# BauerLab/VARSCOT

Hardware: AMD Instinct MI355X
Metric: guides/sec (candidate sites/sec alongside) at <=8 mismatches on a 3.0 Gbp reference (higher is better)
Workload: dtype u32

## Files before the change

varscot_amd/csrc/vsc_api.cpp:

```cpp
#include <algorithm>
#include <atomic>
#include <chrono>
#include <cstdlib>
#include <cmath>
#include <cstdio>
#include <cstring>
#include <memory>
#include <new>
#include <string>
#include <vector>

#include "vsc_bulge.h"
#include "vsc_efficiency.h"
#include "vsc_pattern.h"
#include "vsc_pattern_enum.h"
#include "vsc_pattern_bulge.h"
#include "vsc_enum.h"
#include "vsc_internal.h"
#include "vsc_objects.h"
#include "vsc_pairs.h"
#include "vsc_pick_device.h"
#include "vsc_sites.h"
#include "vsc_bulge_table.h"
#include "vsc_table.h"
// ... 1275 lines not shown
                double e2 = 0;
                for (int left = 0; left <= (int)m; ++left) e2 += (double)left_reads[c][left] * neighbours(left - k0 - k1 - 2);
                const double per_list = e2 / kBucketsPerSeg;
                bytes += (1.0 - std::exp(-per_list)) * (double)genome->ix_class_sites[c] * block_bytes;
                visits += per_list * (double)genome->ix_class_chunks[c] / kSegments;
            }
            for (int k : {k0, k1}) {
                const double per_list = (double)reads_any * neighbours(k) / kBucketsPerSeg;
                bytes += (1.0 - std::exp(-per_list)) * sites_all * block_bytes;
                visits += per_list * chunks_all;
            }
            cost[cut] = std::max(bytes / 4.2e12, visits * 215.0 / ((double)n_cus * 4 * 2.0e9));
        }
        int best = -1;
        for (int cut = 0; cut < 9; ++cut)
            if (cost[cut] >= 0 && (best < 0 || cost[cut] < cost[best])) best = cut;
        const int forced = dbg.seed_tight >= 1 ? dbg.seed_tight - 1 : -1;
        if (forced >= 0 && forced < 9 && cost[forced] >= 0) best = forced;
        if (best < 0) best = 4 * (int)(m ? (m - 1) / kSegments : 0u);
        plan.k0 = (uint32_t)(best % 3);
        plan.k1 = (uint32_t)(best / 3);
        *k2_max = std::min<int>(2, (int)m - (int)plan.k0 - (int)plan.k1 - 2);
    }
    plan.n_nbr = neighbours(std::max<int>(std::max<int>((int)plan.k0, (int)plan.k1), *k2_max));
    return plan;
}

hipError_t seed_plan(vsc_ctx *ctx, const vsc_genome *genome, const uint32_t *gp, uint32_t n_guides, const PassFound &f, SeedArgs &sa,
                     int *n_groups, bool *shared)
{
    int k2_max = 0;
    const SeedPlan plan = seed_cut(genome, gp, n_guides, f.max_mm, ctx->n_cus, ctx->dbg, &k2_max);
    const uint64_t n_pairs = (uint64_t)n_guides * (neighbours((int)plan.k0) + neighbours((int)plan.k1) + plan.n_pam * neighbours(k2_max));
    const uint64_t list_cap = n_pairs + (uint64_t)kLists * (kGuideUnroll - 1) + 2 * kGuideUnroll;
    VSC_TRY(ctx->seed_off.ensure((kLists + 1) * sizeof(uint32_t)));
    VSC_TRY(ctx->seed_poff.ensure((kLists + 1) * sizeof(uint32_t)));
    VSC_TRY(ctx->seed_lrest.ensure(list_cap * sizeof(uint2)));
    VSC_TRY(hipMemsetAsync(ctx->seed_lrest.p, 0xFF, list_cap * sizeof(uint2), ctx->stream));
    VSC_TRY(launch_seed_lists((const uint2 *)ctx->guides.p, n_guides, plan, (uint32_t *)ctx->seed_off.p, (uint32_t *)ctx->seed_poff.p,
                              (uint2 *)ctx->seed_lrest.p, ctx->stream));
    VSC_TRY(hipEventRecord(ctx->ev[kEvPrepEnd], ctx->stream));
    sa.chunk_tab = genome->d_ix_chunk_tab;
    sa.n_chunks = genome->ix_chunks;
    sa.vert = genome->d_ix_vert;
    sa.list_rest = (const uint2 *)ctx->seed_lrest.p;
    sa.sites = genome->d_ix_sites;
    sa.edge_bits = genome->d_ix_edge;
    sa.guides = (const uint2 *)ctx->guides.p;
    sa.poff = (const uint32_t *)ctx->seed_poff.p;
    sa.max_mm = f.max_mm;
    sa.k_half = f.max_mm / 2;
    sa.k_seg0 = plan.k0;
    sa.k_seg1 = plan.k1;
    sa.contig_end = genome->d_contig_end;
    sa.n_contigs = genome->n_contigs;
    sa.counters = (unsigned long long *)ctx->counters.p;
    sa.n_parts = (uint32_t)f.n_parts;
    uint32_t groups_per_cu = kSlicedWavesPerSimd;
    if (ctx->dbg.seed_groups_per_cu) groups_per_cu = ctx->dbg.seed_groups_per_cu;
    *shared = (uint64_t)n_guides * neighbours((int)std::max(plan.k0, plan.k1)) / kBucketsPerSeg >= 72;
    if (ctx->dbg.seed_shared >= 0) *shared = ctx->dbg.seed_shared == 1;
    const uint32_t n_grabs = (sa.n_chunks + kSlicedGrab - 1) / kSlicedGrab;
    const uint32_t n_waves_max = (uint32_t)ctx->n_cus * groups_per_cu * kWavesPerGroup;
    const uint32_t n_waves = std::max<uint32_t>(1, std::min<uint32_t>(n_waves_max, *shared ? n_grabs * kWavesPerGroup : n_grabs));
    *n_groups = (int)((n_waves + kWavesPerGroup - 1) / kWavesPerGroup);
    sa.group_out = *shared && ctx->dbg.seed_group_out != 0 ? 1u : 0u;
    const uint32_t owners = sa.group_out ? (uint32_t)*n_groups : (uint32_t)*n_groups * kWavesPerGroup;
    const uint64_t per_wave = f.cap / ((uint64_t)owners * 8 * f.n_parts);
    uint32_t want_reserve = (uint32_t)std::min<uint64_t>(f.n_parts > 8 ? (sa.group_out ? 1024 : 128) : 1024, std::max<uint64_t>(kWave, per_wave));
    if (ctx->dbg.seed_reserve) want_reserve = std::min<uint32_t>(1024, std::max<uint32_t>(kWave, ctx->dbg.seed_reserve));
    sa.reserve_log2 = 6;
    while ((2u << sa.reserve_log2) <= want_reserve) ++sa.reserve_log2;
    sa.reserve = 1u << sa.reserve_log2;
    sa.pos_pad = f.pos_pad;
    sa.pos_base = f.pos_base;
    uint64_t part_cap = f.cap / f.n_parts + f.cap / f.n_parts / 7 + 4096;
    part_cap = std::max<uint64_t>(part_cap, (uint64_t)(1.2 * genome->seen_rate[f.max_mm] * std::min<uint32_t>(n_guides, kRegionReads)) + 4096);
    sa.part_cap = part_cap + (uint64_t)owners * sa.reserve;
    return hipSuccess;
}

constexpr uint32_t kSeedPartsDefault = 1;
constexpr uint32_t kSeedPartsMax = 64;
constexpr uint32_t kSeedPartGroupsPerCu = 3;
constexpr uint64_t kSeedPartMinRecords = 1ull << 27;

uint32_t plan_parts(vsc_ctx *ctx, const vsc_genome *genome, const PassFound &f, const SeedArgs &sa, uint32_t n_guides, bool shared, SortLevel1 &l1)
{
    const vsc_debug_params &dbg = ctx->dbg;
    uint32_t want = dbg.seed_parts ? dbg.seed_parts : kSeedPartsDefault;
    if (want <= 1 || !shared || ctx->cu_masked || dbg.sort_optimistic == 0 || !genome->sort_slots_ok[f.max_mm]) return 1;
    const double rate = genome->seen_rate[f.max_mm];
    const uint64_t n_max = (uint64_t)(rate * std::min<uint32_t>(n_guides, kRegionReads)), n_all = (uint64_t)(rate * n_guides);
    want = std::min<uint32_t>({want, std::max<uint32_t>(1, sa.n_chunks), kSeedPartsMax});
    if (!dbg.seed_parts && n_all < (uint64_t)want * kSeedPartMinRecords) return 1;
    uint64_t sort_cap, slot_cap;
    unsigned max_bits;
    sort_limits(dbg, &sort_cap, &max_bits, &slot_cap);
    unsigned bits = level_bits(n_max, sort_cap, max_bits, f.key_bits, (size_t)f.n_parts);
    if (bits == 0) {
        if (!dbg.seed_parts) return 1;
        bits = 1;
    }
    if (dbg.sort_optimistic != 1 && !slots_fit((uint64_t)f.n_parts << bits, slot_cap, std::max<uint64_t>(n_all, 1), ctx->keys_b.cap, 0, false)) return 1;
    l1.bits = bits;
    l1.slot_cap = slot_cap;
    return want;
}

size_t round256(size_t n) { return (n + 255) / 256 * 256; }

hipError_t search_in_parts(vsc_ctx *ctx, PassFound &f, const SeedArgs &all, uint32_t K, bool shared, unsigned long long *cnt, size_t cnt_bytes,
                           uint32_t *list_total, float *scan_ms)
{
    const hipStream_t A = ctx->stream;
    SeedArgs sa = all;
    const uint32_t R = (uint32_t)f.n_parts;
    const size_t cnt_at = 0, segs_at = round256(cnt_bytes), tile_at = segs_at + round256(R * sizeof(SortSeg));
    const size_t stride = tile_at + round256((R + 1) * sizeof(uint32_t)), dev_stride = stride - segs_at;
    if (!ctx->stream_b) VSC_TRY(hipStreamCreateWithFlags(&ctx->stream_b, hipStreamNonBlocking));
    const hipStream_t B = ctx->stream_b;
    while (ctx->part_ev.size() < 3 * (size_t)K + 1) {
        hipEvent_t e = nullptr;
        VSC_TRY(hipEventCreate(&e));
        ctx->part_ev.push_back(e);
    }
    if (ctx->pinned_cap < K * stride + 256) {
        if (ctx->pinned) (void)hipHostFree(ctx->pinned);
        ctx->pinned = nullptr;
        ctx->pinned_cap = 0;
        VSC_TRY(hipHostMalloc(&ctx->pinned, K * stride + 256, hipHostMallocDefault));
        ctx->pinned_cap = K * stride + 256;
    }
    char *const pin = (char *)ctx->pinned;
    uint32_t *const pin_total = (uint32_t *)(pin + K * stride);
    SortLevel1 &l1 = f.l1;
    const size_t n_bins = (size_t)R << l1.bits;
    VSC_TRY(ctx->keys_b.ensure(std::max<uint64_t>((uint64_t)n_bins * l1.slot_cap, f.cap) * sizeof(uint64_t)));
    VSC_TRY(ctx->sort_tabs.ensure(3 * n_bins * sizeof(uint32_t)));
    VSC_TRY(ctx->sort_over.ensure(256 + n_bins * sizeof(SortSeg)));
    VSC_TRY(ctx->sort_segs.ensure(std::max<size_t>(K * dev_stride, round256(R * sizeof(SortSeg)) + (R + 1) * sizeof(uint32_t))));
    SortArgs pa{};
    pa.n_segs = R;
    pa.in = (const uint64_t *)ctx->keys_a.p;
    pa.out = (uint64_t *)ctx->keys_b.p;
    pa.cursor = (uint32_t *)ctx->sort_tabs.p + n_bins;
    pa.hist = pa.cursor;
    pa.bin_start = pa.cursor + n_bins;
    pa.bin_bits = l1.bits;
    pa.bin_shift = kRecPosShift + f.pos_pad + f.key_bits - l1.bits;
    pa.fill = l1.fill;
    pa.fill_shift = l1.fill_shift;
    pa.slot_cap = (uint32_t)l1.slot_cap;
    pa.overflow = (uint32_t *)ctx->sort_over.p + 2;
    VSC_TRY(hipMemsetAsync(pa.cursor, 0, n_bins * sizeof(uint32_t), A));
    VSC_TRY(hipMemsetAsync(ctx->sort_over.p, 0, 3 * sizeof(uint32_t), A));
    VSC_TRY(hipMemcpyAsync(pin_total, (const uint32_t *)ctx->seed_poff.p + kLists, sizeof(uint32_t), hipMemcpyDeviceToHost, A));
    VSC_TRY(hipEventRecord(ctx->ev[kEvSearchStart], A));
    for (uint32_t i = 0; i < K; ++i) {
        const uint32_t chunk_first = (uint32_t)((uint64_t)all.n_chunks * i / K);
        sa.chunk_tab = all.chunk_tab + chunk_first;
        sa.n_chunks = (uint32_t)((uint64_t)all.n_chunks * (i + 1) / K) - chunk_first;
        const uint32_t per_cu = ctx->dbg.seed_groups_per_cu ? ctx->dbg.seed_groups_per_cu : (i ? kSeedPartGroupsPerCu : (uint32_t)kSlicedWavesPerSimd);
        const uint32_t n_grabs = (sa.n_chunks + kSlicedGrab - 1) / kSlicedGrab;
        const uint32_t n_waves = std::max<uint32_t>(1, std::min<uint32_t>((uint32_t)ctx->n_cus * per_cu * kWavesPerGroup, shared ? n_grabs * kWavesPerGroup : n_grabs));
        if (i) VSC_TRY(hipMemsetAsync(sa.counters + kCursorBase, 0, (size_t)kCursors * kCursorStride * sizeof(unsigned long long), A));
        VSC_TRY(hipEventRecord(ctx->part_ev[3 * i], A));
        VSC_TRY(launch_seed_sliced(sa, (int)((n_waves + kWavesPerGroup - 1) / kWavesPerGroup), shared, A));
        VSC_TRY(hipEventRecord(ctx->part_ev[3 * i + 1], A));
        VSC_TRY(hipMemcpyAsync(pin + i * stride + cnt_at, sa.counters, cnt_bytes, hipMemcpyDeviceToHost, A));
        VSC_TRY(hipEventRecord(ctx->part_ev[3 * i + 2], A));
    }
    VSC_TRY(hipEventRecord(ctx->ev[kEvSearchEnd], A));
    bool lost = false;
    for (uint32_t i = 0; i < K; ++i) {
        VSC_TRY(hipEventSynchronize(ctx->part_ev[3 * i + 2]));
        const unsigned long long *const now = (const unsigned long long *)(pin + i * stride + cnt_at);
        const unsigned long long *const before = i ? (const unsigned long long *)(pin + (i - 1) * stride + cnt_at) : nullptr;
        if (now[kCntOverflow]) lost = true;
        if (lost) continue;
        SortSeg *const segs = (SortSeg *)(pin + i * stride + segs_at);
        uint32_t *const tile0 = (uint32_t *)(pin + i * stride + tile_at);
        uint64_t tiles = 0;
        for (uint32_t q = 0; q < R; ++q) {
            const uint64_t b = before ? before[kCntPart + 4 * q] : 0, e = now[kCntPart + 4 * q];
            const uint64_t at = (uint64_t)q * sa.part_cap + b;
            segs[q] = SortSeg{at, at, 0, (uint32_t)(e - b), 0, q, 0};
            tile0[q] = (uint32_t)tiles;
            tiles += (e - b + kSortTile - 1) / kSortTile;
        }
        tile0[R] = (uint32_t)tiles;
        if (tiles == 0) continue;
        if (tiles >= (1ull << 31)) return hipErrorInvalidValue;
        char *const dev = (char *)ctx->sort_segs.p + i * dev_stride;
        VSC_TRY(hipStreamWaitEvent(B, ctx->part_ev[3 * i + 2], 0));
        VSC_TRY(hipMemcpyAsync(dev, segs, dev_stride, hipMemcpyHostToDevice, B));
        pa.segs = (const SortSeg *)dev;
        pa.seg_tile0 = (const uint32_t *)(dev + (tile_at - segs_at));
        pa.n_tiles = (uint32_t)tiles;
        pa.xcd_tiles = 0;
        pa.xcd_by_region = 0;
        if (ctx->dbg.sort_xcd != 0 && tiles >= 64) {
            pa.xcd_by_region = 1;
            for (uint32_t x = 0; x <= 8; ++x) pa.xcd_first[x] = tile0[(uint64_t)R * x / 8];
            for (uint32_t x = 0; x < 8; ++x) pa.xcd_tiles = std::max(pa.xcd_tiles, pa.xcd_first[x + 1] - pa.xcd_first[x]);
        }
        VSC_TRY(launch_bin_partition(pa, B));
    }
    VSC_TRY(hipEventRecord(ctx->part_ev[3 * K], B));
    VSC_TRY(hipStreamWaitEvent(A, ctx->part_ev[3 * K], 0));
    std::memcpy(cnt, pin + (K - 1) * stride + cnt_at, cnt_bytes);
    *list_total = *pin_total;
    *scan_ms = 0;
    for (uint32_t i = 0; i < K; ++i) {
        float ms = 0;
        VSC_TRY(hipEventElapsedTime(&ms, ctx->part_ev[3 * i], ctx->part_ev[3 * i + 1]));
        *scan_ms += ms;
    }
    l1.done = !lost;
    if (lost) VSC_TRY(hipStreamSynchronize(A));
    return hipSuccess;
}

int find_pass(vsc_ctx *ctx, const vsc_genome *genome, const uint64_t *guides, uint32_t n_guides, uint32_t guide_base,
              const vsc_search_params *params, bool keep_bases, bool sort_only, vsc_timing &t, PassFound &f)
{
    const int algo = (int)t.algorithm;
    const uint32_t m = params->max_mismatches;
    f.algo = algo;
    f.max_mm = m;
    f.guide_base = guide_base;
    f.bases = keep_bases;
    const uint32_t n_pad = (n_guides + kGuideUnroll - 1) / kGuideUnroll * kGuideUnroll;
    std::vector<uint32_t> gp((size_t)(n_pad + kGuideUnroll) * 2, 0xFFFFFFFFu);
    for (uint32_t i = 0; i < n_guides; ++i) guide_planes(guides[i], &gp[2 * (size_t)i], &gp[2 * (size_t)i + 1]);
    VSC_HIP(ctx, ctx->guides.ensure(gp.size() * sizeof(uint32_t)));
    VSC_HIP(ctx, ctx->counters.ensure(kCounterWords * sizeof(unsigned long long)));
    VSC_HIP(ctx, hipEventRecord(ctx->ev[kEvPassStart], ctx->stream));
    VSC_HIP(ctx, hipMemcpyAsync(ctx->guides.p, gp.data(), gp.size() * sizeof(uint32_t), hipMemcpyHostToDevice, ctx->stream));

    const double own_bases = (double)genome->n_tiles * kTileBases;
    const double sites_est = genome->sites ? (double)genome->sites : own_bases / 4;
    f.cap = (uint64_t)(1.5 * sites_est * n_guides * hit_probability(m)) + (1u << 20);
    const double seen_rate = genome->seen_rate[m];
    if (algo == VSC_ALGO_SCAN) f.cap = std::max<uint64_t>(f.cap, (uint64_t)(1.2 * seen_rate * n_guides) + 4096);
    unsigned long long cnt[kCntPart + 4 * kParts] = {};
    f.n_parts = (int)((n_guides + kRegionReads - 1) / kRegionReads);
    f.pos_base = (uint32_t)(genome->first_word * 32);
    const unsigned pos_bits = std::max(1u, ceil_log2((uint64_t)genome->dev_words * 32));
    f.pos_pad = pos_bits < 32 ? 32 - pos_bits : 0;
    f.key_bits = pos_bits + 1 + ceil_log2(std::min<uint32_t>(n_guides, kRegionReads));

    ScanArgs a{};
    SeedArgs sa{};
    int n_groups = 1;
    bool seed_shared = false;
    const bool use_fill = algo == VSC_ALGO_SEED && sort_only && !keep_bases;
    uint32_t n_parts_k = 1;
    auto owners_of = [](const SeedArgs &s, int groups) { return (uint64_t)(s.group_out ? groups : groups * kWavesPerGroup); };
    if (algo == VSC_ALGO_SCAN) {
        fill_pam(a, params);
        fill_genome(a, ctx, genome);
        a.guides = (const uint4 *)ctx->guides.p;
        a.n_guides_padded = n_pad;
        a.max_mm = m;
        a.k_half = m / 2;
        n_groups = scan_groups(ctx, a.n_tiles);
        t.genome_bytes += (uint64_t)genome->n_tiles * kTileWords * 3 * sizeof(uint32_t);
        VSC_HIP(ctx, hipEventRecord(ctx->ev[kEvPrepEnd], ctx->stream));
    } else {
        VSC_HIP(ctx, seed_plan(ctx, genome, gp.data(), n_guides, f, sa, &n_groups, &seed_shared));
        if (use_fill) {
// ... 7073 lines not shown
```

varscot_amd/csrc/vsc_internal.h:

```cpp
#pragma once

#include <hip/hip_runtime.h>
#include <stdint.h>

#include "varscot_hip.h"
#include "vsc_efficiency.h"
#include "vsc_eff_trees.h"
#include "vsc_mh.h"
#include "vsc_fold.h"
#include "vsc_edit.h"
#include "vsc_variation.h"
#include "vsc_prime.h"
#include "vsc_hdr.h"
#include "vsc_effects.h"

namespace vsc {

constexpr int kWave = 64;
constexpr int kWavesPerGroup = 4;
constexpr int kSitesPerLane = 8;
constexpr int kBatch = kWave * kSitesPerLane;
constexpr int kQueueCap = kBatch + kWave;
constexpr int kHitCap = 128;
constexpr int kTileWords = kWave;
constexpr int kTileBases = kTileWords * 32;
constexpr int kChunkTiles = 8;
constexpr int kGuideUnroll = 4;
constexpr uint32_t kMask23 = 0x7FFFFFu;
constexpr int kSiteStrandBit = 23;
constexpr int kSiteEdgeBit = 24;
constexpr uint32_t kPadWords = 4;

constexpr int kSegments = 3;
constexpr int kSegBases = 7;
constexpr int kBucketsPerSeg = 1 << (2 * kSegBases);
constexpr int kBuckets = kSegments * kBucketsPerSeg;
constexpr int kSeedHitCap = 256;
constexpr int kSlicedSites = 32;
constexpr int kSlicedChunk = kWave * kSlicedSites;
constexpr int kRestBases = VSC_READ_LEN - kSegBases;
constexpr int kCmpBases = 2 * kSegBases;
constexpr int kVertWords = 2 * kCmpBases;
constexpr int kSeedClasses = 3;
constexpr int kLists = (kSegments - 1 + kSeedClasses) * kBucketsPerSeg;
constexpr int kListBudgetShift = 16;
constexpr uint32_t kListNoBudget = 15;
constexpr int kTokLaneShift = 26;
constexpr int kTokSlotShift = 14;
constexpr uint32_t kTokReadMask = (1u << kTokSlotShift) - 1u;
constexpr int kSlicedResolve = 3;
constexpr int kSlicedTokCap = 512;
constexpr uint32_t kChunkBucketMask = 0xFFFFu;
constexpr int kChunkMinusShift = 16;
constexpr int kChunkEdgeBit = 28;
constexpr int kChunkClassShift = 29;
constexpr uint32_t kIndexLayout = 2;
constexpr int kSlicedWavesPerSimd = 6;
constexpr int kSlicedGrab = 8;

enum { kCntHits = 0, kCntChunk = 1, kCntSites = 2, kCntOverflow = 3, kCntVisited = 4, kCntPad = 5, kCntLost = 6, kCntGroups = 7, kCntSlots = 8 };
constexpr int kRegionBits = 6;
constexpr int kRegionReads = 1 << kRegionBits;
constexpr int kParts = 256;
constexpr int kMaxPassReads = kParts * kRegionReads;
constexpr int kCntPart = 8;
constexpr int kCursors = 32;
constexpr int kCursorStride = 16;
constexpr int kCursorBase = kCntPart + 4 * kParts + 8;
constexpr int kCounterWords = kCursorBase + kCursors * kCursorStride;

constexpr int kRecPosShift = 23;
constexpr int kRecStrandShift = 55;
constexpr int kRecReadShift = 56;
constexpr int kRecKeyBits = 33 + kRegionBits;
constexpr uint64_t kRecSentinel = ~0ull;

constexpr int kSortThreads = 512;
constexpr int kSortItems = 16;
constexpr int kSortTile = kSortThreads * kSortItems;
constexpr int kFinThreads = 512;
constexpr int kFinItems = 16;
constexpr int kSortCap = kFinThreads * kFinItems - 128;
constexpr int kSortMaxBinBits = 11;
constexpr int kSortSubBits = 13;
constexpr int kSortSubBitsRows = 12;
constexpr int kHistTiles = 8;

struct PamMasks {
    uint32_t ah, al;
    uint32_t bh, bl;
};

struct ScanArgs {
    const uint32_t *hi, *lo, *nm;
    uint32_t first_pos;
    uint32_t n_tiles;
    const uint4 *guides;
    uint32_t n_guides_padded;
    uint32_t max_mm;
    uint32_t k_half;
    uint32_t n_pam;
    PamMasks pam[3];
    const uint32_t *contig_end;
    uint32_t n_contigs;
    uint64_t *hit_keys;
    uint32_t *hit_vals;
    unsigned long long hit_cap;
    unsigned long long *counters;
    uint32_t *site_x, *site_l, *site_pos;
};

struct SortSeg {
    uint64_t in_off;
    uint64_t out_off;
    uint64_t final_off;
    uint32_t n_in;
    uint32_t guide_base;
    uint32_t region = 0;
    uint32_t pad = 0;
};

struct SortArgs {
    const SortSeg *segs;
    const uint32_t *seg_tile0;
    uint32_t n_segs, n_tiles;
    const uint64_t *in;
    const uint64_t *pair_keys;
    const uint32_t *pair_vals;
    uint64_t *out;
    const uint32_t *side_in;
    uint32_t *side_out;
    uint32_t *hist;
    uint32_t *cursor;
    uint32_t *bin_start;
    uint32_t bin_bits, bin_shift;
    uint32_t pos_pad;
    uint32_t pos_base;
    uint32_t xcd_tiles;
    uint32_t xcd_by_region;
    uint32_t xcd_first[9];
    const uint32_t *fill;
    uint32_t fill_shift;
    uint32_t slot_cap;
    uint32_t *overflow;
};

struct FinArgs {
    const SortSeg *segs;
    uint32_t n_segs;
    const uint64_t *src;
    const uint32_t *hist;
    const uint32_t *bin_start;
    uint32_t bin_bits;
    uint32_t sub_shift, sub_bits;
    uint32_t low_bits;
    uint32_t pos_pad;
    uint32_t pos_base;
    SortSeg *over;
    uint32_t over_cap;
    uint32_t cap;
    uint32_t *n_over;
    uint32_t *cursor;
    const uint32_t *contig_off;
    uint32_t n_contigs;
    vsc_hit *out;
    uint32_t slot_cap;
    const uint32_t *overflow;
    const uint32_t *side_src;
    const uint2 *guides;
    uint32_t guide_first;
    uint4 *rows;
    uint64_t rows_first;
};

struct ScoreArgs {
    const vsc_hit *hits;
    uint64_t n;
    const uint2 *hl;
    uint32_t first_pos;
    uint64_t n_plane_words;
    const uint32_t *contig_off;
    const uint2 *guides;
    double *mit;
    uint8_t *mit_flags;
    uint8_t *features;
    const uint64_t *seg_prefix;
    const uint64_t *seg_start;
    uint32_t n_segs;
};

struct SeedPlan {
    uint32_t max_mm, k0, k1, tight;
    uint32_t n_nbr;
    uint32_t n_pam;
    uint32_t pam_codes;
};

struct SeedArgs {
    const uint4 *chunk_tab;
    const uint32_t *vert;
    const uint2 *list_rest;
    const uint2 *sites;
    const uint32_t *edge_bits;
    const uint2 *guides;
    uint32_t n_chunks;
    const uint32_t *poff;
    uint32_t max_mm, k_half;
    uint32_t k_seg0, k_seg1;
    const uint32_t *contig_end;
    uint32_t n_contigs;
    uint64_t *hit_recs;
    uint32_t *hit_side;
    uint32_t group_out;
    uint32_t reserve;
    uint32_t reserve_log2;
    uint32_t pos_pad;
    uint32_t pos_base;
    uint32_t n_parts;
    unsigned long long part_cap;
    unsigned long long *counters;
    uint32_t *fill;
};

constexpr int kSumThreads = 256;
constexpr int kSumItems = 8;
constexpr int kSumTile = kSumThreads * kSumItems;
constexpr int kSumTilesPerBlock = 8;
// ... 569 lines not shown
```

varscot_amd/csrc/vsc_sort.hip:

```cpp
#include "vsc_internal.h"
#include "vsc_device.h"

namespace vsc {

namespace {

constexpr int kLaneRun = 2;
__device__ __forceinline__ uint32_t tile_record(int k, uint32_t t)
{
    return (uint32_t)(k / kLaneRun) * (uint32_t)(kLaneRun * kSortThreads) + t * (uint32_t)kLaneRun + (uint32_t)(k % kLaneRun);
}

template <int kThreads>
__device__ __forceinline__ uint32_t block_exclusive_scan(uint32_t *s, uint32_t n, uint32_t *s_wave)
{
    const uint32_t t = threadIdx.x, lane = t % kWave, wave = t / kWave;
    const uint32_t per = n > (uint32_t)kThreads ? n / kThreads : 1u;
    const bool mine = t * per < n;
    uint32_t v[4] = {0u, 0u, 0u, 0u};
    uint32_t sum = 0;
    if (mine)
        for (uint32_t i = 0; i < per; ++i) {
            v[i] = s[t * per + i];
            sum += v[i];
        }
    uint32_t inc = sum;
#pragma unroll
    for (int d = 1; d < kWave; d <<= 1) {
        const uint32_t o = __shfl_up(inc, d, kWave);
        if (lane >= (uint32_t)d) inc += o;
    }
    if (lane == kWave - 1) s_wave[wave] = inc;
    block_sync();
    uint32_t before = 0, total = 0;
#pragma unroll
    for (int w = 0; w < kThreads / kWave; ++w) {
        const uint32_t x = s_wave[w];
        before += (uint32_t)w < wave ? x : 0u;
        total += x;
    }
    uint32_t run = before + inc - sum;
    if (mine)
        for (uint32_t i = 0; i < per; ++i) {
            s[t * per + i] = run;
            run += v[i];
        }
    block_sync();
    return total;
}

__device__ __forceinline__ bool slot_filled(const SortArgs &a, uint64_t at, uint32_t held)
{
    return ((uint32_t)at & ((1u << a.fill_shift) - 1u)) < held;
}

__device__ __forceinline__ uint64_t pack_pair(uint64_t key, uint32_t val, uint32_t pos_pad, uint32_t pos_base)
{
    const uint64_t high = (key >> 32) & ((1ull << (kRecKeyBits - 32)) - 1ull);
    return (((high << 32) | (uint32_t)(((uint32_t)key - pos_base) << pos_pad)) << kRecPosShift) | (val & kMask23);
}

}

template <bool kPairs, bool kFill = false>
__global__ __launch_bounds__(kSortThreads) void bin_hist_kernel(const SortArgs a)
{
    __shared__ uint32_t s_hist[1 << kSortMaxBinBits];
    const uint32_t t = threadIdx.x;
    const uint32_t nbins = 1u << a.bin_bits;
    for (uint32_t b = t; b < nbins; b += kSortThreads) s_hist[b] = 0;
    block_sync();
    const uint32_t tile_begin = blockIdx.x * kHistTiles, tile_end = min(tile_begin + (uint32_t)kHistTiles, a.n_tiles);
    uint32_t seg = segment_of_tile(a.seg_tile0, a.n_segs, tile_begin);
    for (uint32_t tile = tile_begin; tile < tile_end; ++tile) {
        if (tile >= a.seg_tile0[seg + 1]) {
            block_sync();
            for (uint32_t b = t; b < nbins; b += kSortThreads) {
                const uint32_t c = s_hist[b];
                if (c) atomicAdd(&a.hist[((size_t)a.segs[seg].region << a.bin_bits) + b], c);
                s_hist[b] = 0;
            }
            block_sync();
            seg = segment_of_tile(a.seg_tile0, a.n_segs, tile);
        }
        const SortSeg sg = a.segs[seg];
        const uint32_t first = (tile - a.seg_tile0[seg]) * (uint32_t)kSortTile;
        const uint32_t n = min(sg.n_in - first, (uint32_t)kSortTile);
        uint64_t r[kSortItems];
        uint32_t held[kFill ? kSortItems / kLaneRun : 1];
        if (kFill) {
#pragma unroll
            for (int j = 0; j < kSortItems / kLaneRun; ++j) {
                const uint32_t i = tile_record(j * kLaneRun, t);
                held[j] = a.fill[(sg.in_off + first + (i < n ? i : 0u)) >> a.fill_shift];
            }
        }
#pragma unroll
        for (int k = 0; k < kSortItems; ++k) {
            const uint32_t i = tile_record(k, t);
            const bool valid = i < n && (!kFill || slot_filled(a, sg.in_off + first + i, held[kFill ? k / kLaneRun : 0]));
            const uint64_t at = sg.in_off + first + (valid ? i : 0u);
            const uint64_t v = kPairs ? a.pair_keys[at] : a.in[at];
            r[k] = valid ? v : kRecSentinel;
        }
#pragma unroll
        for (int k = 0; k < kSortItems; ++k) {
            if (kPairs) {
                if (tile_record(k, t) < n) atomicAdd(&s_hist[(uint32_t)(r[k] >> a.bin_shift)], 1u);
            } else {
                if (!(r[k] >> 63)) atomicAdd(&s_hist[(uint32_t)(r[k] >> a.bin_shift) & (nbins - 1u)], 1u);
            }
        }
    }
    block_sync();
    for (uint32_t b = t; b < nbins; b += kSortThreads) {
        const uint32_t c = s_hist[b];
        if (c) atomicAdd(&a.hist[((size_t)a.segs[seg].region << a.bin_bits) + b], c);
    }
}

hipError_t launch_bin_hist(const SortArgs &args, hipStream_t stream)
{
    if (args.n_tiles == 0) return hipSuccess;
    const unsigned blocks = (args.n_tiles + kHistTiles - 1) / kHistTiles;
    if (args.pair_keys)
        hipLaunchKernelGGL(bin_hist_kernel<true>, dim3(blocks), dim3(kSortThreads), 0, stream, args);
    else if (args.fill)
        hipLaunchKernelGGL((bin_hist_kernel<false, true>), dim3(blocks), dim3(kSortThreads), 0, stream, args);
    else
        hipLaunchKernelGGL(bin_hist_kernel<false>, dim3(blocks), dim3(kSortThreads), 0, stream, args);
    return hipGetLastError();
}

__global__ __launch_bounds__(512) void bin_scan_kernel(const SortArgs a)
{
    __shared__ uint32_t s_cnt[1 << kSortMaxBinBits];
    __shared__ uint32_t s_wave[512 / kWave];
    const uint32_t nbins = 1u << a.bin_bits;
    const size_t base = (size_t)blockIdx.x << a.bin_bits;
    for (uint32_t b = threadIdx.x; b < nbins; b += 512) s_cnt[b] = a.hist[base + b];
    block_sync();
    block_exclusive_scan<512>(s_cnt, nbins, s_wave);
    for (uint32_t b = threadIdx.x; b < nbins; b += 512) {
        a.bin_start[base + b] = s_cnt[b];
        if (!a.slot_cap) a.cursor[base + b] = s_cnt[b];
    }
}

hipError_t launch_bin_scan(const SortArgs &args, hipStream_t stream)
{
    if (args.n_segs == 0) return hipSuccess;
    hipLaunchKernelGGL(bin_scan_kernel, dim3(args.n_segs), dim3(512), 0, stream, args);
    return hipGetLastError();
}

template <bool kPairs, bool kSide = false, bool kFill = false>
__global__ __launch_bounds__(kSortThreads) void bin_partition_kernel(const SortArgs a)
{
    __shared__ uint64_t s_rec[kSortTile];
    __shared__ uint32_t s_cnt[(1 << kSortMaxBinBits) + kWave];
    __shared__ uint32_t s_gbase[kPairs ? (1 << kSortMaxBinBits) : 1];
    __shared__ uint32_t s_over[(1 << kSortMaxBinBits) / 32 + 1];
    __shared__ uint32_t s_wave[kSortThreads / kWave];
    const uint32_t t = threadIdx.x;
    const uint32_t nbins = 1u << a.bin_bits;
    uint32_t tile = blockIdx.x;
    if (a.xcd_by_region) {
        tile = a.xcd_first[blockIdx.x & 7u] + (blockIdx.x >> 3);
        if (tile >= a.xcd_first[(blockIdx.x & 7u) + 1u]) return;
    } else if (a.xcd_tiles) {
        tile = (blockIdx.x & 7u) * a.xcd_tiles + (blockIdx.x >> 3);
        if ((blockIdx.x >> 3) >= a.xcd_tiles || tile >= a.n_tiles) return;
    }
    const uint32_t seg = segment_of_tile(a.seg_tile0, a.n_segs, tile);
    const SortSeg sg = a.segs[seg];
    const uint32_t first = (tile - a.seg_tile0[seg]) * (uint32_t)kSortTile;
    const uint32_t n = min(sg.n_in - first, (uint32_t)kSortTile);
    uint32_t held[kFill ? kSortItems / kLaneRun : 1];
    if (kFill) {
#pragma unroll
        for (int j = 0; j < kSortItems / kLaneRun; ++j) {
            const uint32_t i = tile_record(j * kLaneRun, t);
            held[j] = a.fill[(sg.in_off + first + (i < n ? i : 0u)) >> a.fill_shift];
        }
    }
    for (uint32_t b = t; b < nbins + kWave; b += kSortThreads) s_cnt[b] = 0;
    for (uint32_t b = t; b < (1u << kSortMaxBinBits) / 32u + 1u; b += kSortThreads) s_over[b] = 0;
    block_sync();
    uint64_t r[kSortItems];
    uint32_t bin[kSortItems];
    uint32_t side[kSide ? kSortItems : 1];
#pragma unroll
    for (int k = 0; k < kSortItems; ++k) {
        const uint32_t i = tile_record(k, t);
        const bool in_tile = i < n && (!kFill || slot_filled(a, sg.in_off + first + i, held[kFill ? k / kLaneRun : 0]));
        const uint64_t at = sg.in_off + first + (in_tile ? i : 0u);
        if (kSide) side[k] = a.side_in[at];
        if (kPairs) {
            const uint64_t key = a.pair_keys[at];
            r[k] = in_tile ? pack_pair(key, a.pair_vals[at], a.pos_pad, a.pos_base) : kRecSentinel;
            bin[k] = in_tile ? (uint32_t)(key >> a.bin_shift) : 0u;
        } else {
            const uint64_t v = a.in[at];
            r[k] = in_tile ? v : kRecSentinel;
            bin[k] = (uint32_t)(r[k] >> a.bin_shift) & (nbins - 1u);
        }
    }
    const uint32_t spare = nbins + (t % kWave);
#pragma unroll
    for (int k = 0; k < kSortItems; ++k) {
        const bool real = !(r[k] >> 63);
        const uint32_t rank = atomicAdd(&s_cnt[real ? bin[k] : spare], real ? 1u : 0u);
        bin[k] |= rank << 16;
    }
    block_sync();
    constexpr int kOwnBins = (1 << kSortMaxBinBits) / kSortThreads;
    uint32_t own_at[kOwnBins];
#pragma unroll
    for (int j = 0; j < kOwnBins; ++j) {
        const uint32_t b = t + (uint32_t)j * kSortThreads;
        const uint32_t c = b < nbins ? s_cnt[b] : 0u;
        uint32_t at = c ? atomicAdd(&a.cursor[((size_t)sg.region << a.bin_bits) + b], c) : 0u;
        if (a.slot_cap && c && at + c > a.slot_cap) {
            atomicOr(a.overflow, 1u);
            atomicOr(&s_over[b >> 5], 1u << (b & 31u));
            s_over[(1u << kSortMaxBinBits) / 32u] = 1u;
        }
        own_at[j] = at;
        if (kPairs && b < nbins) s_gbase[b] = at;
    }
    const uint32_t total = block_exclusive_scan<kSortThreads>(s_cnt, nbins, s_wave);
#pragma unroll
    for (int k = 0; k < kSortItems; ++k) {
        const uint32_t slot = s_cnt[bin[k] & 0xFFFFu] + (bin[k] >> 16);
        if (!(r[k] >> 63)) s_rec[slot] = r[k];
        if (kSide) bin[k] = slot;
    }
    block_sync();
    if (!kPairs) {
#pragma unroll
        for (int j = 0; j < kOwnBins; ++j) {
            const uint32_t b = t + (uint32_t)j * kSortThreads;
            if (b < nbins) s_cnt[b] = own_at[j] - s_cnt[b];
        }
        block_sync();
    }
    const bool any_over = s_over[(1u << kSortMaxBinBits) / 32u] != 0u;
    uint32_t slot_bin[kSide ? kSortItems / 2 : 1];
    if (kSide) {
#pragma unroll
        for (int j = 0; j < kSortItems / 2; ++j) slot_bin[j] = 0;
    }
    for (uint32_t i = t; i < total; i += kSortThreads) {
        const uint64_t x = s_rec[i];
        uint32_t b;
        if (kPairs) {
            uint32_t lo = 0, hi = nbins;
            while (hi - lo > 1) {
                const uint32_t mid = (lo + hi) >> 1;
                if (s_cnt[mid] <= i) lo = mid; else hi = mid;
            }
            b = lo;
        } else {
            b = (uint32_t)(x >> a.bin_shift) & (nbins - 1u);
        }
        const uint32_t in_bin = kPairs ? s_gbase[b] + (i - s_cnt[b]) : s_cnt[b] + i;
        const bool skip = any_over && ((s_over[b >> 5] >> (b & 31u)) & 1u);
        if (a.slot_cap) {
            if (!skip) a.out[(((uint64_t)sg.region << a.bin_bits) + b) * a.slot_cap + in_bin] = x;
        } else {
            a.out[sg.out_off + in_bin] = x;
        }
        if (kSide) {
            const uint32_t j = i / kSortThreads;
#pragma unroll
            for (int q = 0; q < kSortItems / 2; ++q)
                if ((uint32_t)q == (j >> 1)) slot_bin[q] |= b << ((j & 1u) * 16u);
        }
    }
    if (kSide) {
        block_sync();
        uint32_t *const s_side = (uint32_t *)s_rec;
#pragma unroll
        for (int k = 0; k < kSortItems; ++k)
            if (!(r[k] >> 63)) s_side[bin[k]] = side[k];
        block_sync();
#pragma unroll
        for (int j = 0; j < kSortItems; ++j) {
            const uint32_t i = t + (uint32_t)j * kSortThreads;
            if (i < total) {
                const uint32_t b = (slot_bin[j >> 1] >> ((j & 1) * 16)) & 0xFFFFu;
                const uint32_t in_bin = s_cnt[b] + i;
                const bool skip = any_over && ((s_over[b >> 5] >> (b & 31u)) & 1u);
                if (a.slot_cap) {
                    if (!skip) a.side_out[(((uint64_t)sg.region << a.bin_bits) + b) * a.slot_cap + in_bin] = s_side[i];
                } else {
                    a.side_out[sg.out_off + in_bin] = s_side[i];
                }
            }
        }
    }
}

hipError_t launch_bin_partition(const SortArgs &args, hipStream_t stream)
{
    if (args.n_tiles == 0) return hipSuccess;
    const unsigned blocks = args.xcd_tiles ? 8u * args.xcd_tiles : args.n_tiles;
    if (args.pair_keys)
        hipLaunchKernelGGL(bin_partition_kernel<true>, dim3(blocks), dim3(kSortThreads), 0, stream, args);
    else if (args.side_in)
        hipLaunchKernelGGL((bin_partition_kernel<false, true>), dim3(blocks), dim3(kSortThreads), 0, stream, args);
    else if (args.fill)
        hipLaunchKernelGGL((bin_partition_kernel<false, false, true>), dim3(blocks), dim3(kSortThreads), 0, stream, args);
    else
        hipLaunchKernelGGL(bin_partition_kernel<false>, dim3(blocks), dim3(kSortThreads), 0, stream, args);
    return hipGetLastError();
}

__global__ __launch_bounds__(256) void fill_holes_kernel(const SortSeg *segs, uint64_t *recs, const uint32_t *fill, uint32_t fill_shift)
{
    const SortSeg sg = segs[blockIdx.x];
    const uint32_t lane = threadIdx.x % kWave, wave = threadIdx.x / kWave, block = 1u << fill_shift;
    for (uint32_t b0 = wave * block; b0 < sg.n_in; b0 += (256 / kWave) * block) {
        const uint32_t held = min(fill[(sg.in_off + b0) >> fill_shift], block);
        for (uint32_t i = held + lane; i < block && b0 + i < sg.n_in; i += kWave) recs[sg.in_off + b0 + i] = kRecSentinel;
    }
}

hipError_t launch_fill_holes(const SortSeg *segs, uint32_t n_segs, uint64_t *recs, const uint32_t *fill, uint32_t fill_shift, hipStream_t stream)
{
    if (n_segs == 0) return hipSuccess;
    hipLaunchKernelGGL(fill_holes_kernel, dim3(n_segs), dim3(256), 0, stream, segs, recs, fill, fill_shift);
    return hipGetLastError();
}

__device__ __forceinline__ uint32_t sub_slot(const uint32_t *s_sub, uint32_t sb)
{
    return (s_sub[sb >> 1] >> ((sb & 1u) * 16u)) & 0xFFFFu;
}

constexpr int kFinalizeAhead = 4;
constexpr int kFinalizeNear = 4;
constexpr int kFinalizeRange = 64;

template <bool kRows>
__device__ __forceinline__ void finalize_bin(const FinArgs &a, const uint32_t which)
{
    __shared__ uint64_t s_rec[kSortCap];
    __shared__ uint32_t s_sub[(1 << (kRows ? kSortSubBitsRows : kSortSubBits)) / 2 + 1 + kWave];
    __shared__ uint4 s_stage[kRows ? (kFinThreads / kWave) * 64 : 1];
    __shared__ uint32_t s_wave[kFinThreads / kWave];
    __shared__ uint32_t s_range[2 + kFinalizeRange];
    __shared__ uint32_t s_edge[4];
    uint32_t t_ = threadIdx.x;
    asm volatile("" : "+v"(t_));
    const uint32_t t = t_;
    const uint32_t seg = which >> a.bin_bits, bin = which & ((1u << a.bin_bits) - 1u);
    const SortSeg sg = a.segs[seg];
    uint64_t src = sg.in_off, dst = sg.final_off;
    uint64_t compact = sg.in_off;
    uint32_t n_src = sg.n_in;
    if (a.hist) {
        const size_t idx = ((size_t)seg << a.bin_bits) + bin;
        n_src = a.hist[idx];
        const uint32_t st = a.bin_start[idx];
        src = a.slot_cap ? (uint64_t)idx * a.slot_cap : sg.out_off + st;
        dst = sg.final_off + st;
        compact = sg.in_off + st;
    }
    if (n_src == 0) return;
    if (n_src > a.cap) {
        if (t == 0) {
            const uint32_t slot = atomicAdd(a.n_over, 1u);
            if (slot < a.over_cap) {
                SortSeg o;
                o.in_off = src;
                o.out_off = a.slot_cap ? compact : src;
                o.final_off = dst;
                o.n_in = n_src;
                o.guide_base = sg.guide_base;
                o.region = 0;
                o.pad = 0;
                a.over[slot] = o;
            }
        }
        return;
    }
    const uint32_t nsub = 1u << a.sub_bits;
    const uint32_t nwords = nsub > 1u ? nsub / 2u : 1u;
    for (uint32_t i = t; i <= nwords + kWave; i += kFinThreads) s_sub[i] = 0;
// ... 344 lines not shown
```

Baseline: 284,100.

## Add slim bin-partition kernel to co-run beside seed search parts

Adds a small-footprint variant of the bin partition kernel (256 threads, 8 items, capped VGPRs, reduced LDS) used for all but the last seed part. It is sized so two of its workgroups fit on a CU alongside search workgroups, so partitioning on stream B can overlap the next part's search. The slim path also simplifies bin extraction to the high word and drops the per-record fill check in favour of a block-level count. The search groups per CU for later parts rise from 3 to 5 to match. The risk is that a smaller tile raises per-tile overhead and global cursor atomics, and co-residency may slow the search.

```diff
diff --git a/varscot_amd/csrc/vsc_api.cpp b/varscot_amd/csrc/vsc_api.cpp
--- a/varscot_amd/csrc/vsc_api.cpp
+++ b/varscot_amd/csrc/vsc_api.cpp
@@ -1381,7 +1381,7 @@
 
 constexpr uint32_t kSeedPartsDefault = 1;
 constexpr uint32_t kSeedPartsMax = 64;
-constexpr uint32_t kSeedPartGroupsPerCu = 3;
+constexpr uint32_t kSeedPartGroupsPerCu = 5;
 constexpr uint64_t kSeedPartMinRecords = 1ull << 27;
 
 uint32_t plan_parts(vsc_ctx *ctx, const vsc_genome *genome, const PassFound &f, const SeedArgs &sa, uint32_t n_guides, bool shared, SortLevel1 &l1)
@@ -1452,6 +1452,7 @@
     pa.fill_shift = l1.fill_shift;
     pa.slot_cap = (uint32_t)l1.slot_cap;
     pa.overflow = (uint32_t *)ctx->sort_over.p + 2;
+    const bool slim_ok = pa.bin_shift >= 32 && (l1.slot_cap << l1.bits) < (1ull << 32);
     VSC_TRY(hipMemsetAsync(pa.cursor, 0, n_bins * sizeof(uint32_t), A));
     VSC_TRY(hipMemsetAsync(ctx->sort_over.p, 0, 3 * sizeof(uint32_t), A));
     VSC_TRY(hipMemcpyAsync(pin_total, (const uint32_t *)ctx->seed_poff.p + kLists, sizeof(uint32_t), hipMemcpyDeviceToHost, A));
@@ -1480,13 +1481,15 @@
         if (lost) continue;
         SortSeg *const segs = (SortSeg *)(pin + i * stride + segs_at);
         uint32_t *const tile0 = (uint32_t *)(pin + i * stride + tile_at);
+        pa.slim = i + 1 < K && slim_ok ? 1u : 0u;
+        const uint64_t tile = pa.slim ? kSortSlimTile : kSortTile;
         uint64_t tiles = 0;
         for (uint32_t q = 0; q < R; ++q) {
             const uint64_t b = before ? before[kCntPart + 4 * q] : 0, e = now[kCntPart + 4 * q];
             const uint64_t at = (uint64_t)q * sa.part_cap + b;
             segs[q] = SortSeg{at, at, 0, (uint32_t)(e - b), 0, q, 0};
             tile0[q] = (uint32_t)tiles;
-            tiles += (e - b + kSortTile - 1) / kSortTile;
+            tiles += (e - b + tile - 1) / tile;
         }
         tile0[R] = (uint32_t)tiles;
         if (tiles == 0) continue;
diff --git a/varscot_amd/csrc/vsc_internal.h b/varscot_amd/csrc/vsc_internal.h
--- a/varscot_amd/csrc/vsc_internal.h
+++ b/varscot_amd/csrc/vsc_internal.h
@@ -78,6 +78,10 @@
 constexpr int kSortThreads = 512;
 constexpr int kSortItems = 16;
 constexpr int kSortTile = kSortThreads * kSortItems;
+constexpr int kSortSlimThreads = 256;
+constexpr int kSortSlimItems = 8;
+constexpr int kSortSlimTile = kSortSlimThreads * kSortSlimItems;
+static_assert(kSortTile % kSortSlimTile == 0, "part_cap and the fill table's blocks are multiples of kSortTile: a slim tile must not straddle regions");
 constexpr int kFinThreads = 512;
 constexpr int kFinItems = 16;
 constexpr int kSortCap = kFinThreads * kFinItems - 128;
@@ -143,6 +147,7 @@
     uint32_t fill_shift;
     uint32_t slot_cap;
     uint32_t *overflow;
+    uint32_t slim;
 };
 
 struct FinArgs {
diff --git a/varscot_amd/csrc/vsc_sort.hip b/varscot_amd/csrc/vsc_sort.hip
--- a/varscot_amd/csrc/vsc_sort.hip
+++ b/varscot_amd/csrc/vsc_sort.hip
@@ -6,18 +6,19 @@
 namespace {
 
 constexpr int kLaneRun = 2;
+template <int kThreads = kSortThreads>
 __device__ __forceinline__ uint32_t tile_record(int k, uint32_t t)
 {
-    return (uint32_t)(k / kLaneRun) * (uint32_t)(kLaneRun * kSortThreads) + t * (uint32_t)kLaneRun + (uint32_t)(k % kLaneRun);
-}
-
-template <int kThreads>
+    return (uint32_t)(k / kLaneRun) * (uint32_t)(kLaneRun * kThreads) + t * (uint32_t)kLaneRun + (uint32_t)(k % kLaneRun);
+}
+
+template <int kThreads, int kMaxPer = 4>
 __device__ __forceinline__ uint32_t block_exclusive_scan(uint32_t *s, uint32_t n, uint32_t *s_wave)
 {
     const uint32_t t = threadIdx.x, lane = t % kWave, wave = t / kWave;
     const uint32_t per = n > (uint32_t)kThreads ? n / kThreads : 1u;
     const bool mine = t * per < n;
-    uint32_t v[4] = {0u, 0u, 0u, 0u};
+    uint32_t v[kMaxPer] = {};
     uint32_t sum = 0;
     if (mine)
         for (uint32_t i = 0; i < per; ++i) {
@@ -154,14 +155,26 @@
     return hipGetLastError();
 }
 
-template <bool kPairs, bool kSide = false, bool kFill = false>
-__global__ __launch_bounds__(kSortThreads) void bin_partition_kernel(const SortArgs a)
-{
-    __shared__ uint64_t s_rec[kSortTile];
-    __shared__ uint32_t s_cnt[(1 << kSortMaxBinBits) + kWave];
-    __shared__ uint32_t s_gbase[kPairs ? (1 << kSortMaxBinBits) : 1];
-    __shared__ uint32_t s_over[(1 << kSortMaxBinBits) / 32 + 1];
-    __shared__ uint32_t s_wave[kSortThreads / kWave];
+template <bool kPairs, int kThreads, int kItems>
+struct PartitionLds {
+    uint64_t rec[kThreads * kItems];
+    uint32_t cnt[(1 << kSortMaxBinBits) + kWave];
+    uint32_t gbase[kPairs ? (1 << kSortMaxBinBits) : 1];
+    uint32_t over[(1 << kSortMaxBinBits) / 32 + 1];
+    uint32_t wave[kThreads / kWave];
+};
+static_assert(sizeof(PartitionLds<false, kSortSlimThreads, kSortSlimItems>) <= 29440, "slim: two workgroups per CU beside five of the search");
+static_assert(sizeof(PartitionLds<false, kSortThreads, kSortItems>) <= 163840 / 2, "two workgroups per CU");
+
+template <bool kPairs, bool kSide, bool kFill, int kThreads, int kItems>
+__device__ __forceinline__ void bin_partition_tile(const SortArgs &a, PartitionLds<kPairs, kThreads, kItems> &lds)
+{
+    constexpr int kTile = kThreads * kItems;
+    constexpr bool kSlim = kThreads != kSortThreads;
+    static_assert(!kSlim || (kFill && !kPairs && !kSide), "the slim shape: fill table and slot mode only");
+    static_assert(kTile <= (1 << 16) && (1 << kSortMaxBinBits) % kThreads == 0, "a tile's ranks fit 16 bits; whole bins per thread");
+    uint64_t *const s_rec = lds.rec;
+    uint32_t *const s_cnt = lds.cnt, *const s_gbase = lds.gbase, *const s_over = lds.over, *const s_wave = lds.wave;
     const uint32_t t = threadIdx.x;
     const uint32_t nbins = 1u << a.bin_bits;
     uint32_t tile = blockIdx.x;
@@ -174,84 +187,133 @@
     }
     const uint32_t seg = segment_of_tile(a.seg_tile0, a.n_segs, tile);
     const SortSeg sg = a.segs[seg];
-    const uint32_t first = (tile - a.seg_tile0[seg]) * (uint32_t)kSortTile;
-    const uint32_t n = min(sg.n_in - first, (uint32_t)kSortTile);
-    uint32_t held[kFill ? kSortItems / kLaneRun : 1];
+    const uint32_t first = (tile - a.seg_tile0[seg]) * (uint32_t)kTile;
+    const uint32_t n = min(sg.n_in - first, (uint32_t)kTile);
+    uint32_t held[kFill ? kItems / kLaneRun : 1];
     if (kFill) {
 #pragma unroll
-        for (int j = 0; j < kSortItems / kLaneRun; ++j) {
-            const uint32_t i = tile_record(j * kLaneRun, t);
+        for (int j = 0; j < kItems / kLaneRun; ++j) {
+            const uint32_t i = tile_record<kThreads>(j * kLaneRun, t);
             held[j] = a.fill[(sg.in_off + first + (i < n ? i : 0u)) >> a.fill_shift];
         }
     }
-    for (uint32_t b = t; b < nbins + kWave; b += kSortThreads) s_cnt[b] = 0;
-    for (uint32_t b = t; b < (1u << kSortMaxBinBits) / 32u + 1u; b += kSortThreads) s_over[b] = 0;
-    block_sync();
-    uint64_t r[kSortItems];
-    uint32_t bin[kSortItems];
-    uint32_t side[kSide ? kSortItems : 1];
-#pragma unroll
-    for (int k = 0; k < kSortItems; ++k) {
-        const uint32_t i = tile_record(k, t);
-        const bool in_tile = i < n && (!kFill || slot_filled(a, sg.in_off + first + i, held[kFill ? k / kLaneRun : 0]));
-        const uint64_t at = sg.in_off + first + (in_tile ? i : 0u);
-        if (kSide) side[k] = a.side_in[at];
-        if (kPairs) {
-            const uint64_t key = a.pair_keys[at];
-            r[k] = in_tile ? pack_pair(key, a.pair_vals[at], a.pos_pad, a.pos_base) : kRecSentinel;
-            bin[k] = in_tile ? (uint32_t)(key >> a.bin_shift) : 0u;
-        } else {
-            const uint64_t v = a.in[at];
-            r[k] = in_tile ? v : kRecSentinel;
-            bin[k] = (uint32_t)(r[k] >> a.bin_shift) & (nbins - 1u);
+    for (uint32_t b = t; b < nbins + kWave; b += kThreads) s_cnt[b] = 0;
+    for (uint32_t b = t; b < (1u << kSortMaxBinBits) / 32u + 1u; b += kThreads) s_over[b] = 0;
+    block_sync();
+    uint64_t r[kItems];
+    uint32_t bin[kItems];
+    uint32_t side[kSide ? kItems : 1];
+    if constexpr (kSlim) {
+        const uint32_t in_block = (1u << a.fill_shift) - 1u, high_shift = a.bin_shift - 32u;
+        const uint64_t *const in = a.in + sg.in_off + first;
+#pragma unroll
+        for (int j = 0; j < kItems / kLaneRun; ++j) {
+            const uint32_t i = tile_record<kThreads>(j * kLaneRun, t);
+            const int there = min((int)min(held[j], in_block + 1u) - (int)(i & in_block), (int)n - (int)i);
+#pragma unroll
+            for (int q = 0; q < kLaneRun; ++q) {
+                const int k = j * kLaneRun + q;
+                const bool in_tile = q < there;
+                const uint64_t v = in[in_tile ? i + (uint32_t)q : 0u];
+                r[k] = in_tile ? v : kRecSentinel;
+                bin[k] = ((uint32_t)(r[k] >> 32) >> high_shift) & (nbins - 1u);
+            }
+        }
+    } else {
+#pragma unroll
+        for (int k = 0; k < kItems; ++k) {
+            const uint32_t i = tile_record<kThreads>(k, t);
+            const bool in_tile = i < n && (!kFill || slot_filled(a, sg.in_off + first + i, held[kFill ? k / kLaneRun : 0]));
+            const uint64_t at = sg.in_off + first + (in_tile ? i : 0u);
+            if (kSide) side[k] = a.side_in[at];
+            if (kPairs) {
+                const uint64_t key = a.pair_keys[at];
+                r[k] = in_tile ? pack_pair(key, a.pair_vals[at], a.pos_pad, a.pos_base) : kRecSentinel;
+                bin[k] = in_tile ? (uint32_t)(key >> a.bin_shift) : 0u;
+            } else {
+                const uint64_t v = a.in[at];
+                r[k] = in_tile ? v : kRecSentinel;
+                bin[k] = (uint32_t)(r[k] >> a.bin_shift) & (nbins - 1u);
+            }
         }
     }
     const uint32_t spare = nbins + (t % kWave);
 #pragma unroll
-    for (int k = 0; k < kSortItems; ++k) {
+    for (int k = 0; k < kItems; ++k) {
         const bool real = !(r[k] >> 63);
         const uint32_t rank = atomicAdd(&s_cnt[real ? bin[k] : spare], real ? 1u : 0u);
         bin[k] |= rank << 16;
     }
     block_sync();
-    constexpr int kOwnBins = (1 << kSortMaxBinBits) / kSortThreads;
-    uint32_t own_at[kOwnBins];
-#pragma unroll
-    for (int j = 0; j < kOwnBins; ++j) {
-        const uint32_t b = t + (uint32_t)j * kSortThreads;
-        const uint32_t c = b < nbins ? s_cnt[b] : 0u;
-        uint32_t at = c ? atomicAdd(&a.cursor[((size_t)sg.region << a.bin_bits) + b], c) : 0u;
+    constexpr int kOwnBins = (1 << kSortMaxBinBits) / kThreads;
+    auto reserve = [&](uint32_t b, uint32_t c) {
+        const uint32_t at = c ? atomicAdd(&a.cursor[((size_t)sg.region << a.bin_bits) + b], c) : 0u;
         if (a.slot_cap && c && at + c > a.slot_cap) {
             atomicOr(a.overflow, 1u);
             atomicOr(&s_over[b >> 5], 1u << (b & 31u));
             s_over[(1u << kSortMaxBinBits) / 32u] = 1u;
         }
-        own_at[j] = at;
-        if (kPairs && b < nbins) s_gbase[b] = at;
-    }
-    const uint32_t total = block_exclusive_scan<kSortThreads>(s_cnt, nbins, s_wave);
-#pragma unroll
-    for (int k = 0; k < kSortItems; ++k) {
+        return at;
+    };
+    uint32_t own_at[kSlim ? 1 : kOwnBins];
+    if constexpr (!kSlim) {
+#pragma unroll
+        for (int j = 0; j < kOwnBins; ++j) {
+            const uint32_t b = t + (uint32_t)j * kThreads;
+            own_at[j] = reserve(b, b < nbins ? s_cnt[b] : 0u);
+            if (kPairs && b < nbins) s_gbase[b] = own_at[j];
+        }
+    }
+    const uint32_t total = block_exclusive_scan<kThreads, (kOwnBins > 4 ? kOwnBins : 4)>(s_cnt, nbins, s_wave);
+#pragma unroll
+    for (int k = 0; k < kItems; ++k) {
         const uint32_t slot = s_cnt[bin[k] & 0xFFFFu] + (bin[k] >> 16);
         if (!(r[k] >> 63)) s_rec[slot] = r[k];
         if (kSide) bin[k] = slot;
     }
     block_sync();
-    if (!kPairs) {
+    if constexpr (kSlim) {
+        uint32_t first_slot[kOwnBins], count[kOwnBins];
 #pragma unroll
         for (int j = 0; j < kOwnBins; ++j) {
-            const uint32_t b = t + (uint32_t)j * kSortThreads;
+            const uint32_t b = t + (uint32_t)j * kThreads;
+            first_slot[j] = b < nbins ? s_cnt[b] : 0u;
+            count[j] = b < nbins ? (b + 1u < nbins ? s_cnt[b + 1u] : total) - first_slot[j] : 0u;
+        }
+        block_sync();
+#pragma unroll
+        for (int j = 0; j < kOwnBins; ++j) {
+            const uint32_t b = t + (uint32_t)j * kThreads;
+            const uint32_t at = reserve(b, count[j]);
+            if (b < nbins) s_cnt[b] = at - first_slot[j] + b * a.slot_cap;
+        }
+        block_sync();
+    } else if (!kPairs) {
+#pragma unroll
+        for (int j = 0; j < kOwnBins; ++j) {
+            const uint32_t b = t + (uint32_t)j * kThreads;
             if (b < nbins) s_cnt[b] = own_at[j] - s_cnt[b];
         }
         block_sync();
     }
     const bool any_over = s_over[(1u << kSortMaxBinBits) / 32u] != 0u;
-    uint32_t slot_bin[kSide ? kSortItems / 2 : 1];
+    uint32_t slot_bin[kSide ? kItems / 2 : 1];
     if (kSide) {
 #pragma unroll
-        for (int j = 0; j < kSortItems / 2; ++j) slot_bin[j] = 0;
-    }
-    for (uint32_t i = t; i < total; i += kSortThreads) {
+        for (int j = 0; j < kItems / 2; ++j) slot_bin[j] = 0;
+    }
+    if constexpr (kSlim) {
+        uint64_t *const out = a.out + ((uint64_t)sg.region << a.bin_bits) * a.slot_cap;
+        const uint32_t high_shift = a.bin_shift - 32u;
+        for (uint32_t i = t; i < total; i += kThreads) {
+            const uint64_t x = s_rec[i];
+            const uint32_t b = ((uint32_t)(x >> 32) >> high_shift) & (nbins - 1u);
+            const bool skip = any_over && ((s_over[b >> 5] >> (b & 31u)) & 1u);
+            if (!skip) out[s_cnt[b] + i] = x;
+        }
+        return;
+    }
+    for (uint32_t i = t; i < total; i += kThreads) {
         const uint64_t x = s_rec[i];
         uint32_t b;
         if (kPairs) {
@@ -272,9 +334,9 @@
             a.out[sg.out_off + in_bin] = x;
         }
         if (kSide) {
-            const uint32_t j = i / kSortThreads;
-#pragma unroll
-            for (int q = 0; q < kSortItems / 2; ++q)
+            const uint32_t j = i / kThreads;
+#pragma unroll
+            for (int q = 0; q < kItems / 2; ++q)
                 if ((uint32_t)q == (j >> 1)) slot_bin[q] |= b << ((j & 1u) * 16u);
         }
     }
@@ -282,12 +344,12 @@
         block_sync();
         uint32_t *const s_side = (uint32_t *)s_rec;
 #pragma unroll
-        for (int k = 0; k < kSortItems; ++k)
+        for (int k = 0; k < kItems; ++k)
             if (!(r[k] >> 63)) s_side[bin[k]] = side[k];
         block_sync();
 #pragma unroll
-        for (int j = 0; j < kSortItems; ++j) {
-            const uint32_t i = t + (uint32_t)j * kSortThreads;
+        for (int j = 0; j < kItems; ++j) {
+            const uint32_t i = t + (uint32_t)j * kThreads;
             if (i < total) {
                 const uint32_t b = (slot_bin[j >> 1] >> ((j & 1) * 16)) & 0xFFFFu;
                 const uint32_t in_bin = s_cnt[b] + i;
@@ -302,10 +364,30 @@
     }
 }
 
+template <bool kPairs, bool kSide = false, bool kFill = false>
+__global__ __launch_bounds__(kSortThreads) void bin_partition_kernel(const SortArgs a)
+{
+    __shared__ PartitionLds<kPairs, kSortThreads, kSortItems> lds;
+    bin_partition_tile<kPairs, kSide, kFill, kSortThreads, kSortItems>(a, lds);
+}
+
+using SlimLds = PartitionLds<false, kSortSlimThreads, kSortSlimItems>;
+__global__ __launch_bounds__(kSortSlimThreads) __attribute__((amdgpu_num_vgpr(28))) void bin_partition_slim_kernel(const SortArgs a)
+{
+    extern __shared__ uint64_t slim_lds[];
+    bin_partition_tile<false, false, true, kSortSlimThreads, kSortSlimItems>(a, *reinterpret_cast<SlimLds *>(slim_lds));
+}
+
 hipError_t launch_bin_partition(const SortArgs &args, hipStream_t stream)
 {
     if (args.n_tiles == 0) return hipSuccess;
     const unsigned blocks = args.xcd_tiles ? 8u * args.xcd_tiles : args.n_tiles;
+    if (args.slim) {
+        if (args.pair_keys || args.side_in || !args.fill || !args.slot_cap || args.bin_shift < 32 || ((uint64_t)args.slot_cap << args.bin_bits) >= (1ull << 32))
+            return hipErrorInvalidValue;
+        hipLaunchKernelGGL(bin_partition_slim_kernel, dim3(blocks), dim3(kSortSlimThreads), sizeof(SlimLds), stream, args);
+        return hipGetLastError();
+    }
     if (args.pair_keys)
         hipLaunchKernelGGL(bin_partition_kernel<true>, dim3(blocks), dim3(kSortThreads), 0, stream, args);
     else if (args.side_in)
```

After: 276,900. 0.975x the previous value.
